# rikuu/Gap2Seq

Hardware: AMD Instinct MI355X
Metric: gaps filled/sec (whole node), k=31 synthetic 3 Mbp DBG (higher is better)
Workload: dtype u32

## Files before the change

gap2seq_amd/csrc/d3_device.h:

```cpp
#pragma once
#include <hip/hip_runtime_api.h>
#include <stdint.h>

#include "d2_device.h"
#include "fill_device.h"

#define G2S_D3_BLOCK_VARS 16u
#define G2S_RAND_BLOCK 4096u
#define G2S_RAND_WINDOW 160u
#define G2S_D3_TABLE_BUDGET (8u << 20)

#define G2S_D3_UNHANDLED 0x1u
#define G2S_D3_BUDGET 0x2u
#define G2S_D3_ANOMALY 0x4u

namespace g2s {

struct D3Gap {
  uint64_t arena_off;
  int32_t skip_thr;
  uint16_t lmf;
  uint8_t kind;
  uint8_t pad;
};
// ... 32 lines not shown
static_assert(sizeof(D3Var) == 64 && sizeof(D3Trace) == 32, "record layouts");

struct D3Summary {
  uint32_t status, unhandled, n_var, anomalies;
  unsigned long long host_items, host_segs, host_rnd;
  uint32_t handoff_waves, tiles;
  uint64_t table_entries, block_entries;
  uint64_t draws_min, draws_spread, draws_total;
  uint64_t xA, sA, xB, sB, xD, sD, segs, fill_bytes;
  uint32_t seg_gaps, filled;
  uint32_t rand_state[31];
  uint32_t trace_waves;
  uint32_t big_gaps;
  uint32_t traced_gaps;
  uint32_t spec_gaps;
};
static_assert(sizeof(D3Summary) <= 512, "the lap stamps live at byte 512 of the summary's slot");

struct RandTables {
  const uint32_t* hi = nullptr;
  const uint32_t* mid = nullptr;
  const uint32_t* lane = nullptr;
};
void rand_tables_host(uint32_t* hi , uint32_t* mid , uint32_t* lane );

struct D3Work {
  uint32_t* ginfo = nullptr;
  uint32_t* dmin = nullptr;
  uint32_t* dspread = nullptr;
  uint32_t* base = nullptr;
// ... 62 lines not shown
                     const D3Gap* dgaps, const SubRec* sub, const char* lastch_up, const char* lastch_dn,
                     const RandTables& rt, uint32_t* rnd_all ,
                     uint64_t rnd_capacity, void* results ,
                     char* arena , const D3Side& side ,
                     void* summary_host ,
                     bool summary_is_clean ,
                     uint32_t* clean_words ,
                     hipEvent_t ev_chain = nullptr ,
                     hipEvent_t ev_d2 = nullptr ,
                     hipEvent_t ev_stop = nullptr );

hipError_t test_d3_tables(const uint32_t* segs, uint32_t nsegs, int32_t n_len, int32_t len0, int32_t len1, uint32_t start_seg,
                          const uint32_t* rnd, uint64_t rnd_cap, uint32_t base, uint32_t R, uint32_t dmin, uint32_t dspread,
                          uint16_t* entries, uint8_t* bad, uint32_t* anomalies);

}
```

gap2seq_amd/csrc/d3_device.hip:

```cpp
#include "sync_debug.h"
#include <hip/hip_runtime.h>
#include <hip/hip_ext.h>

#include <algorithm>
#include <cstddef>
#include <cstdlib>
#include <cstring>
#include <mutex>
#include <set>
#include <vector>

#include "../../include/g2s.h"
#include "d3_device.h"
#include "envcache.hpp"

namespace {

using g2s::D3Gap;
using g2s::D3Params;
using g2s::D3Summary;
using g2s::D3Work;

__device__ __forceinline__ uint32_t uni(uint32_t x) { return (uint32_t)__builtin_amdgcn_readfirstlane((int)x); }

// ... 38 lines not shown
  x = sat_add(x, (uint32_t)__builtin_amdgcn_update_dpp(0, (int)x, 0x143, 0xC, 0xF, false));
  return x;
}
__device__ __forceinline__ uint32_t dpp_sum(uint32_t x) { return (uint32_t)__builtin_amdgcn_readlane((int)dpp_scan_add(x), 63); }
__device__ __forceinline__ unsigned long long wave_add64(unsigned long long v) {
  const unsigned long long lo = dpp_sum((uint32_t)v & 0xFFFFFFu), mid = dpp_sum((uint32_t)(v >> 24) & 0xFFFFFFu), hi = dpp_sum((uint32_t)(v >> 48));
  return lo + (mid << 24) + (hi << 48);
}

__device__ __forceinline__ uint32_t d3_classify_body(const D3Params& P, const D3Work& W, const GapOut* __restrict__ outs,
                                                     const D3Gap* __restrict__ dgaps, uint32_t first, uint32_t stride,
                                                     uint32_t* l_gi, uint32_t* l_dm, uint32_t* l_ds, int32_t* l_sk,
                                                     unsigned long long* red, bool one_wg) {
  const uint32_t n = P.n;
  unsigned long long xA = 0, sA = 0, xB = 0, sB = 0, xD = 0, sD = 0, segs = 0;
  uint32_t unhandled = 0, seg_gaps = 0, big = 0, traced = 0, spec = 0;
  for (uint32_t i = first; i < n; i += stride) {
    const D3Gap dg = dgaps[i];
    const GapOut& go = outs[i];
    const uint32_t flags = go.flags, n_states = go.n_states, n_right = go.n_right, x_right = go.x_right, x_left = go.x_left;
    const uint32_t x_sub = go.x_sub, n_sub = go.n_sub, nseg_b = go.stat[3], dflags = go.dflags, stop0 = go.stop[0], stop1 = go.stop[1];
    const int c_count = go.c_count, n_len = go.n_len, len0 = go.len[0], len1 = go.len[1], reached_j = go.reached_j, count_s = go.count_s;
    const uint32_t n_xl = go.n_xl;
    const uint64_t sub_off = go.sub_off;
    uint32_t gi = 0, dmin = 0, spread = 0;
    if (dg.kind != 0) gi = GI_BAD;
    else {
      if (flags & (G2S_DEV_OVERFLOW_A | G2S_DEV_OVERFLOW_B)) unhandled++;
      else if ((uint64_t)n_states > P.max_states || (uint64_t)n_right > P.max_states) gi = GI_MEM;
      else {
        xA += x_right; sA += n_right; xB += x_left; sB += n_states; xD += x_sub; sD += n_sub;
        segs += nseg_b;
        seg_gaps++;
        if (flags & G2S_DEV_BIG) big++;
        if (dflags & G2S_DEVA_TRACED) traced++;
        if (dflags & G2S_DEVA_SPEC) spec++;
        const bool phase_d = c_count > 0 && n_len > 0;
        const bool by_host = phase_d && !(dflags & (G2S_DEVA_ANALYSED | G2S_DEVA_D2_PENDING));
        const int cnt = (phase_d && !P.skip_confident && P.all_paths) ? count_s : c_count;
        if (cnt > 0 && (!P.unique_paths || cnt == 1)) gi |= GI_FILLED;
        if (n_len > 0) gi |= ((uint32_t)reached_j & 0xFFu) << 8;
        if (phase_d) {
          gi |= GI_PHASE_D;
          if (by_host) gi |= GI_HOST;
          int lo_d = 0x7FFFFFFF, hi_d = 0;
#pragma unroll
          for (int q = 0; q < 2; q++) {
            if (q >= n_len) continue;
            const uint32_t sw = q ? stop1 : stop0;
            const int lq = q ? len1 : len0;
            int lo = (int)(sw & 0xFFFFu), hi = (int)(sw >> 16);
            if (lo > hi || hi > (int)dg.lmf) { lo = 0; hi = (int)dg.lmf; }
            lo_d = min(lo_d, 1 + lq - hi);
            hi_d = max(hi_d, 1 + lq - lo);
          }
          lo_d = max(lo_d, 1);
          hi_d = max(hi_d, lo_d);
          dmin = (uint32_t)lo_d;
          spread = (uint32_t)(hi_d - lo_d);
// ... 10 lines not shown
    uint4 h0;
    const uint64_t ao = P.arena_base + dg.arena_off, sa = (uint64_t)(i / P.group_size) * P.sub_region + sub_off;
    h0.x = (uint32_t)ao; h0.y = (uint32_t)(ao >> 32); h0.z = (uint32_t)sa; h0.w = (uint32_t)(sa >> 32);
    ((uint4*)&W.tdesc[i])[0] = h0;
    (void)n_xl;
  }
  xA = wave_add64(xA); sA = wave_add64(sA); xB = wave_add64(xB); sB = wave_add64(sB); xD = wave_add64(xD); sD = wave_add64(sD);
  segs = wave_add64(segs);
  const unsigned long long cnts = wave_add64(((unsigned long long)unhandled << 32) | seg_gaps);
  big = dpp_sum(big);
  if ((threadIdx.x & 63u) == 0u && big) atomicAdd(&W.sum->big_gaps, big);
  traced = dpp_sum(traced);
  if ((threadIdx.x & 63u) == 0u && traced) atomicAdd(&W.sum->traced_gaps, traced);
  spec = dpp_sum(spec);
  if ((threadIdx.x & 63u) == 0u && spec) atomicAdd(&W.sum->spec_gaps, spec);
  const uint32_t wave = threadIdx.x >> 6, nwaves = blockDim.x >> 6;
  if ((threadIdx.x & 63u) == 0u) {
    unsigned long long* r = red + wave * 8u;
    r[0] = xA; r[1] = sA; r[2] = xB; r[3] = sB; r[4] = xD; r[5] = sD; r[6] = segs; r[7] = cnts;
  }
  __syncthreads();
  unsigned long long tot = 0;
  if (threadIdx.x < 8u) for (uint32_t w = 0; w < nwaves; w++) tot += red[w * 8u + threadIdx.x];
  unsigned long long all_cnts = 0;
  for (uint32_t w = 0; w < nwaves; w++) all_cnts += red[w * 8u + 7u];
  D3Summary* S = W.sum;
  if (threadIdx.x < 7u) {
    unsigned long long* dst = (unsigned long long*)&S->xA + threadIdx.x;
    if (one_wg) *dst = tot; else if (tot) atomicAdd(dst, tot);
  } else if (threadIdx.x == 7u) {
// ... 852 lines not shown
  (void)d3_classify_body(P, W, outs, dgaps, blockIdx.x * 256u + threadIdx.x, gridDim.x * 256u, nullptr, nullptr, nullptr, nullptr, red, false);
  (void)d3_handoff_body<true>(P, W, outs, sub, rnd, capacity, side, blockIdx.x * 256u + (threadIdx.x & ~63u), nullptr, nullptr, nullptr, nullptr);
  if ((threadIdx.x & 63u) == 0u) {
    asm volatile("s_waitcnt vmcnt(0)" ::: "memory");
    const unsigned int done = atomicAdd(&S->handoff_waves, 1u) + 1u;
    if (done == gridDim.x * 4u) {
      const unsigned long long items = atomicAdd(&S->host_items, 0ull);
      const uint32_t anomalies = atomicAdd(&S->anomalies, 0u), unhandled = atomicAdd(&S->unhandled, 0u);
      S->status = unhandled ? G2S_D3_UNHANDLED : 0u;
      __hip_atomic_store(side.count, (items & 0x7FFFFFFFFFFFFFFFull) | ((unsigned long long)((anomalies || unhandled) ? 1u : 0u) << 63),
                         __ATOMIC_RELEASE, __HIP_MEMORY_SCOPE_SYSTEM);
    }
  }
}
#define D3_BACK_TAB 24576u
__global__ __launch_bounds__(1024) void g2s_d3_back(const D3Params P, const D3Work W, const GapOut* __restrict__ outs,
                                                    const SubRec* __restrict__ sub, const uint32_t* __restrict__ Wd, uint64_t capacity,
                                                    const g2s::D3Side side) {
  __shared__ uint32_t total_dev;
  __shared__ unsigned long long lcur[3];
  if (threadIdx.x < 3u) lcur[threadIdx.x] = 0ull;
  __shared__ uint16_t ltab[D3_BACK_TAB];
  __shared__ uint32_t ltoff[1025], ldvar[1025];
  D3Summary* S = W.sum;
  if (threadIdx.x == 0) stamp(W, 8);
  const uint32_t status = S->status, V = S->n_var;
  const uint64_t T = S->table_entries;
  if (status) {
    if (threadIdx.x == 0) __hip_atomic_store(side.count, 1ull << 63, __ATOMIC_RELEASE, __HIP_MEMORY_SCOPE_SYSTEM);
    return;
// ... 31 lines not shown
  for (uint32_t i0 = (threadIdx.x >> 6) * 64u; i0 < P.n; i0 += 1024u)
    (void)d3_handoff_body<false>(P, W, outs, sub, Wd + 31, capacity, side, i0, in_lds ? ldvar : nullptr, in_lds ? ltab : nullptr,
                          in_lds ? ltoff : nullptr, lcur);
  __syncthreads();
  if (threadIdx.x == 0) {
    stamp(W, 11);
    const unsigned long long items = lcur[0];
    S->host_items = items; S->host_segs = lcur[1]; S->host_rnd = lcur[2];
    const uint32_t anomalies = atomicAdd(&S->anomalies, 0u);
    __hip_atomic_store(side.count, (items & 0x7FFFFFFFFFFFFFFFull) | ((unsigned long long)(anomalies ? 1u : 0u) << 63), __ATOMIC_RELEASE,
                       __HIP_MEMORY_SCOPE_SYSTEM);
    stamp(W, 12);
  }
}

template <int NW>
__global__ __launch_bounds__(64 * NW) void g2s_d3_trace(const D3Params P, const D3Work W, GapOut* __restrict__ outs,
                                                   const SubRec* __restrict__ sub, const char* __restrict__ chu,
                                                   const char* __restrict__ chd, const uint32_t* __restrict__ rnd,
                                                   uint64_t capacity, g2s_result* __restrict__ results,
                                                   char* __restrict__ arena, uint32_t* __restrict__ summary_host,
                                                   const g2s::D3Side side, uint32_t* __restrict__ clean_words ) {
  extern __shared__ __attribute__((aligned(16))) uint32_t lds[];
  D3Summary* S = W.sum;
  const uint32_t i = blockIdx.x;
  constexpr int NT = 64 * NW;
  const int tid = (int)threadIdx.x, lane = tid & 63;
  const bool w0 = tid < 64;
#ifdef G2S_SYNC_DEBUG
  auto wg_sync = [&]() { if constexpr (NW > 1) __syncthreads(); else { g2s_sync_jitter(0xD3u); g2s_wait_all(); asm volatile("s_waitcnt lgkmcnt(0)" ::: "memory"); __builtin_amdgcn_wave_barrier(); } };
#else
  auto wg_sync = [&]() { if constexpr (NW > 1) __syncthreads(); else { asm volatile("s_waitcnt lgkmcnt(0)" ::: "memory"); __builtin_amdgcn_wave_barrier(); } };
#endif
  SegW* segs = (SegW*)lds;
  static_assert(sizeof(g2s_result) == 112, "g2s_result layout");
  unsigned long long* laps = (unsigned long long*)((char*)W.sum + 512);
  const unsigned long long tk0 = P.laps ? wall_clock64() : 0ull;
  unsigned long long tk1 = 0, tk2 = 0, tk3 = 0, hops = 0, tkm = 0;
  if (P.laps && i == 0 && tid == 0) laps[13] = tk0;
  const uint32_t status = uni(S->status);
  g2s::D3Trace td;
  {
    const uint4 h0 = ((const uint4*)&W.tdesc[i])[0], h1 = ((const uint4*)&W.tdesc[i])[1];
    td.arena_off = (uint64_t)uni(h0.x) | ((uint64_t)uni(h0.y) << 32);
    td.sub_at = (uint64_t)uni(h0.z) | ((uint64_t)uni(h0.w) << 32);
    td.gi = uni(h1.x); td.off = uni(h1.y); td.want = uni(h1.z);
    td.lmf = (uint16_t)(uni(h1.w) & 0xFFFFu); td.nsegs = (uint16_t)(uni(h1.w) >> 16);
  }
  struct {
    uint32_t flags, dflags, start_seg, start_t, sub_vertices, sub_edges, top_level;
    int32_t c_count, n_len, len[2], reached_j, count_s;
  } go;
  {
    const GapOut& g = outs[i];
    go.top_level = uni(g.top_level);
    go.flags = uni(g.flags); go.dflags = uni(g.dflags); go.start_seg = uni(g.start_seg); go.start_t = uni(g.start_t);
    go.sub_vertices = uni(g.sub_vertices); go.sub_edges = uni(g.sub_edges);
    go.c_count = (int32_t)uni((uint32_t)g.c_count); go.n_len = (int32_t)uni((uint32_t)g.n_len);
    go.len[0] = (int32_t)uni((uint32_t)g.len[0]); go.len[1] = (int32_t)uni((uint32_t)g.len[1]);
    go.reached_j = (int32_t)uni((uint32_t)g.reached_j); go.count_s = (int32_t)uni((uint32_t)g.count_s);
  }
  bool d2_lost = false;
  if ((go.dflags & G2S_DEVA_D2_PENDING) && !(go.dflags & (G2S_DEVA_RUNS | G2S_DEVA_D2_FAILED)) && !P.skip_confident) {
    uint32_t v = go.dflags;
    for (uint32_t spin = 0; spin < (1u << 22) && !(v & (G2S_DEVA_RUNS | G2S_DEVA_D2_FAILED)); spin++) {
      __builtin_amdgcn_s_sleep(8);
      v = uni(__hip_atomic_load(&outs[i].dflags, __ATOMIC_ACQUIRE, __HIP_MEMORY_SCOPE_AGENT));
    }
    __builtin_amdgcn_fence(__ATOMIC_ACQUIRE, "agent");
    go.dflags = v;
    go.sub_vertices = uni(__hip_atomic_load(&outs[i].sub_vertices, __ATOMIC_RELAXED, __HIP_MEMORY_SCOPE_AGENT));
    go.sub_edges = uni(__hip_atomic_load(&outs[i].sub_edges, __ATOMIC_RELAXED, __HIP_MEMORY_SCOPE_AGENT));
    if (!(v & (G2S_DEVA_RUNS | G2S_DEVA_D2_FAILED))) d2_lost = true;
  }
  if ((go.dflags & G2S_DEVA_D2_PENDING) && (go.dflags & G2S_DEVA_D2_FAILED) && !(td.gi & GI_HOST) && (td.gi & GI_PHASE_D)) d2_lost = true;
  uint32_t gsp_all = 0, gsp_sent = 0;
  auto leave = [&](uint32_t fill_len) {
    if (!w0) return;
    uint32_t last = 0;
    if (lane == 0) {
      if (P.laps) {
        const unsigned long long tk4 = wall_clock64();
        atomicMax(&laps[14], tk1 ? tk1 - tk0 : 0ull); atomicMax(&laps[15], tk2 ? tk2 - tk1 : 0ull);
        atomicMax(&laps[16], tk3 ? tk3 - tk2 : 0ull); atomicMax(&laps[17], ((tk4 - tk0) << 24) | ((td.gi & GI_HOST) ? 1ull << 23 : 0ull) | (unsigned long long)(i & 0x7FFFFFu)); atomicMax(&laps[18], tk4);
        atomicMax(&laps[19], ((tk2 ? tk2 - tk1 : 0ull) << 32) | (hops << 16) | (tkm ? tkm - tk1 : 0ull));
        if ((P.laps >> 4) == i + 1u) { laps[26] = tk0; laps[27] = tk1; laps[28] = tkm; laps[29] = tk2; laps[30] = tk3; laps[31] = tk4; }
      }
      const uint32_t c = i & 63u, n = gridDim.x;
// ... 16 lines not shown
    const unsigned long long c1 = __hip_atomic_load(cl + 1, __ATOMIC_RELAXED, __HIP_MEMORY_SCOPE_AGENT);
    summary_host[lane] = s0;
    summary_host[64 + lane] = s1;
    ((unsigned long long*)(summary_host + 256 + 32 * lane))[0] = c0;
    ((unsigned long long*)(summary_host + 256 + 32 * lane))[1] = c1;
    if (P.self_clean) {
      src[lane] = 0u; src[64 + lane] = 0u;
      ((unsigned long long*)(src + 256 + 32 * lane))[0] = 0ull;
      ((unsigned long long*)(src + 256 + 32 * lane))[1] = 0ull;
    }
    if (P.self_clean && clean_words && lane < 32) clean_words[lane] = 0u;
    if (P.laps && lane == 0) { asm volatile("s_waitcnt vmcnt(0)" ::: "memory"); laps[25] = wall_clock64(); }
  };
  if (status) { leave(0u); return; }
  if (d2_lost) {
    if (tid == 0) { atomicAdd(&S->anomalies, 1u); arena[td.arena_off + td.lmf] = '\0'; }
    asm volatile("s_waitcnt vmcnt(0)" ::: "memory");
    leave(0u);
    return;
  }
  const uint32_t gi = td.gi;
  if ((go.dflags & G2S_DEVA_TRACED) && !(gi & (GI_BAD | GI_SKIPPED | GI_MEM | GI_HOST)) && (gi & GI_PHASE_D)) {
    asm volatile("s_waitcnt vmcnt(0)" ::: "memory");
    leave((go.top_level >> 16) - (go.top_level & 0xFFFFu));
    return;
  }
  const bool spec = (go.dflags & G2S_DEVA_SPEC) != 0u && W.spec_text != nullptr && !(gi & (GI_BAD | GI_SKIPPED | GI_MEM | GI_HOST)) && (gi & GI_PHASE_D);
  const int spec_stop = (int)(go.top_level & 0xFFFFu), spec_len = (int)(go.top_level >> 16);
  const unsigned long long spec_chain = spec ? ((unsigned long long)uni(outs[i].stat[6]) | ((unsigned long long)uni(outs[i].stat[7]) << 32)) : 0ull;
  struct { uint16_t lmf; } dg = {td.lmf};
  const uint64_t abs_off = td.arena_off;
// ... 43 lines not shown
    rw[16] = go.sub_vertices; rw[18] = go.sub_edges;
    if (by_runs) {
      const uint4 o0 = ((const uint4*)&W.d2out[i])[0], o1 = ((const uint4*)&W.d2out[i])[1];
      runs = W.d2runs + 2ull * uni(o0.x);
      n_runs = uni(o0.y);
      rw[8] = uni(o0.z); rw[10] = uni(o0.w); rw[12] = uni(o1.x); rw[14] = uni(o1.y); rw[16] = uni(o1.z); rw[18] = uni(o1.w);
    }
  }
  if (!phase_d) {
    if (tid == 0) buf[dg.lmf] = '\0';
    finish(0u);
    leave(0u);
    return;
  }
  if (gi & GI_HOST) {
    const uint32_t it = uni(W.host_slot[i]);
    if (it != 0xFFFFFFFFu) {
      const g2s::D3HostItem* hp = &W.hitems[it];
      const uint64_t so = (uint64_t)uni((uint32_t)hp->seg_off) | ((uint64_t)uni((uint32_t)(hp->seg_off >> 32)) << 32);
      const uint64_t ro = (uint64_t)uni((uint32_t)hp->rnd_off) | ((uint64_t)uni((uint32_t)(hp->rnd_off >> 32)) << 32);
      const uint32_t ns = uni(hp->n_segs), want = uni(hp->draws);
      const GapOut& g = outs[i];
      if ((uint32_t)tid < sizeof(GapOut) / 4u) ((uint32_t*)&side.outs[it])[tid] = ((const uint32_t*)&g)[tid];
      const uint4* src = (const uint4*)(sub + td.sub_at);
      uint4* dst = (uint4*)(side.segs + so);
      for (uint32_t w = (uint32_t)tid; w < 2u * ns; w += (uint32_t)NT) dst[w] = src[w];
      for (uint32_t w = (uint32_t)tid; w < (want + 8u) / 8u; w += (uint32_t)NT) {
        uint32_t pk8 = 0u;
#pragma unroll
        for (uint32_t x = 0; x < 8u; x++) {
          const uint32_t at = 8u * w + x;
          if (at <= want) pk8 |= ((rnd[td.off + at] >> 1) % 12u) << (4u * x);
        }
        side.rnd[ro + w] = pk8;
      }
      __threadfence_system();
// ... 489 lines not shown
  hipLaunchKernelGGL(g2s_d3_blocks, dim3(256), dim3(256), 0, st, W);
  hipLaunchKernelGGL(g2s_d3_groupfn, dim3(std::min(256u, (P.R0 + 256u) / 256u)), dim3(256), 0, st, W, P.R0, group_fn);
  return hipGetLastError();
}
hipError_t launch_d3_sharded_trace(hipStream_t st, const D3Params& P, const D3Work& W, const GapOut* outs, const SubRec* sub,
                                   const char* lastch_up, const char* lastch_dn, uint32_t* rnd_all, uint64_t rnd_capacity,
                                   void* results, char* arena, const D3Side& side, void* summary_host, hipEvent_t ev_d2) {
  if (P.n == 0) return hipSuccess;
  hipLaunchKernelGGL(g2s_d3_chain, dim3(1), dim3(1024), 0, st, W, rnd_all, P.base0, P.d_in);
  if (ev_d2) { const hipError_t e2 = hipStreamWaitEvent(st, ev_d2, 0); if (e2 != hipSuccess) return e2; }
  hipLaunchKernelGGL(g2s_d3_handoff, dim3((P.n + 63u) / 64u), dim3(64), 0, st, P, W, outs, sub, rnd_all + 31, rnd_capacity, side);
  const size_t lds = (size_t)P.seg_cap * (sizeof(SegRec) + 16) + (size_t)P.map_cap * 8 + 16;
  hipError_t e = hipFuncSetAttribute((const void*)g2s_d3_trace<1>, hipFuncAttributeMaxDynamicSharedMemorySize, (int)lds);
  if (e != hipSuccess) return e;
  hipLaunchKernelGGL(g2s_d3_trace<1>, dim3(P.n), dim3(64), lds, st, P, W, const_cast<GapOut*>(outs), sub, lastch_up, lastch_dn, rnd_all + 31, rnd_capacity,
                     (g2s_result*)results, arena, (uint32_t*)summary_host, side, (uint32_t*)nullptr);
  return hipGetLastError();
}

hipError_t launch_d3(hipStream_t st, const D3Params& P, const D3Work& W, const GapDev* gaps, const GapOut* outs,
                     const D3Gap* dgaps, const SubRec* sub, const char* lastch_up, const char* lastch_dn,
                     const RandTables& rt, uint32_t* rnd_all, uint64_t rnd_capacity, void* results, char* arena,
                     const D3Side& side, void* summary_host, bool summary_is_clean, uint32_t* clean_words, hipEvent_t ev_chain,
                     hipEvent_t ev_d2, hipEvent_t ev_stop) {
  if (P.n == 0) return hipSuccess;
  (void)gaps;
  (void)rt;
  static_assert(sizeof(D3Summary) <= 1024, "summary slot");
  hipError_t e = summary_is_clean ? hipSuccess : hipMemsetAsync(W.sum, 0, 1024 + 64 * 128, st);
  if (e != hipSuccess) return e;
  const bool short_list = P.n <= D3_FRONT_GAPS;
  if (P.restart) {
    if (ev_d2) { e = hipStreamWaitEvent(st, ev_d2, 0); if (e != hipSuccess) return e; }
    hipLaunchKernelGGL(g2s_d3_restart, dim3((P.n + 255u) / 256u), dim3(256), 0, st, P, W, outs, dgaps, sub, rnd_all + 31, rnd_capacity, side);
  } else if (short_list) hipLaunchKernelGGL(g2s_d3_front, dim3(1), dim3(1024), 0, st, P, W, outs, dgaps);
  else {
    hipLaunchKernelGGL(g2s_d3_classify, dim3((P.n + 255u) / 256u), dim3(256), 0, st, P, W, outs, dgaps);
    launch_scan(st, P, W, outs);
  }
  if (!P.restart) { e = launch_tables(st, P, W, sub, rnd_all, rnd_capacity); if (e != hipSuccess) return e; }
  if (ev_d2 && short_list && !P.restart) { e = hipStreamWaitEvent(st, ev_d2, 0); if (e != hipSuccess) return e; }
  if (P.restart) (void)ev_chain;
  else if (short_list) {
    hipLaunchKernelGGL(g2s_d3_back, dim3(1), dim3(1024), 0, st, P, W, outs, sub, rnd_all, rnd_capacity, side);
    if (ev_chain) { e = hipEventRecord(ev_chain, st); if (e != hipSuccess) return e; }
  } else {
    hipLaunchKernelGGL(g2s_d3_blocks, dim3(256), dim3(256), 0, st, W);
    hipLaunchKernelGGL(g2s_d3_chain, dim3(1), dim3(1024), 0, st, W, rnd_all, 0u, 0u);
    if (ev_chain) { e = hipEventRecord(ev_chain, st); if (e != hipSuccess) return e; }
    if (ev_d2) { e = hipStreamWaitEvent(st, ev_d2, 0); if (e != hipSuccess) return e; }
    hipLaunchKernelGGL(g2s_d3_handoff, dim3((P.n + 63u) / 64u), dim3(64), 0, st, P, W, outs, sub, rnd_all + 31, rnd_capacity, side);
  }
  const size_t lds = (size_t)P.seg_cap * (sizeof(SegRec) + 16) + (size_t)P.map_cap * 8 + 16;
  const char* waves_s = GENV("G2S_TRACE_WAVES");
  const int waves_env = waves_s ? atoi(waves_s) : 0;
  const bool four = waves_env ? waves_env == 4 : P.n <= 768u;
  e = hipFuncSetAttribute(four ? (const void*)g2s_d3_trace<4> : (const void*)g2s_d3_trace<1>, hipFuncAttributeMaxDynamicSharedMemorySize, (int)lds);
  if (e != hipSuccess) return e;
  if (ev_stop != nullptr) {
    if (four)
      hipExtLaunchKernelGGL(g2s_d3_trace<4>, dim3(P.n), dim3(256), (uint32_t)lds, st, nullptr, ev_stop, 0u, P, W, const_cast<GapOut*>(outs), sub, lastch_up, lastch_dn,
                            rnd_all + 31, rnd_capacity, (g2s_result*)results, arena, (uint32_t*)summary_host, side, clean_words);
    else
      hipExtLaunchKernelGGL(g2s_d3_trace<1>, dim3(P.n), dim3(64), (uint32_t)lds, st, nullptr, ev_stop, 0u, P, W, const_cast<GapOut*>(outs), sub, lastch_up, lastch_dn,
                            rnd_all + 31, rnd_capacity, (g2s_result*)results, arena, (uint32_t*)summary_host, side, clean_words);
    return hipGetLastError();
  }
  if (four)
    hipLaunchKernelGGL(g2s_d3_trace<4>, dim3(P.n), dim3(256), lds, st, P, W, const_cast<GapOut*>(outs), sub, lastch_up, lastch_dn, rnd_all + 31, rnd_capacity,
                       (g2s_result*)results, arena, (uint32_t*)summary_host, side, clean_words);
  else
    hipLaunchKernelGGL(g2s_d3_trace<1>, dim3(P.n), dim3(64), lds, st, P, W, const_cast<GapOut*>(outs), sub, lastch_up, lastch_dn, rnd_all + 31, rnd_capacity,
                       (g2s_result*)results, arena, (uint32_t*)summary_host, side, clean_words);
  return hipGetLastError();
}

}
```

gap2seq_amd/csrc/g2s_api.hip:

```cpp
#include <hip/hip_runtime.h>
#include <cstdarg>
#include <sys/prctl.h>
#include <pthread.h>
#include <sched.h>
#include <time.h>

#include <algorithm>
#include <atomic>
#include <chrono>
#include <cstdio>
#include <cstdlib>
#include <condition_variable>
#include <cstring>
#include <functional>
#include <mutex>
#include <string>
#include <thread>
#include <vector>

#include "../../include/g2s.h"
#include "../../include/g2s_test.h"
#include "envcache.hpp"
#include "d2_device.h"
#include "d3_device.h"
// ... 4761 lines not shown
}

extern "C" int g2s_test_d3_tables(int device, const uint32_t* segs, uint32_t n_segs, int32_t n_len, int32_t len0, int32_t len1,
                                  uint32_t start_seg, const uint32_t* rnd, uint64_t rnd_cap, uint32_t base, uint32_t R, uint32_t dmin,
                                  uint32_t dspread, uint16_t* entries, uint8_t* bad, uint32_t* anomalies) {
  if ((!segs && n_segs) || (!rnd && rnd_cap) || !entries || !bad || !anomalies || n_segs > 0xFFFFu || n_len < 1 || n_len > 2 ||
      (uint64_t)R + 1u > (uint64_t)G2S_D3_TABLE_BUDGET)
    return fail(G2S_ERR_ARG, "g2s_test_d3_tables: bad argument");
  int ndev = 0;
  if (hipGetDeviceCount(&ndev) != hipSuccess || device < 0 || device >= ndev) return fail(G2S_ERR_NO_DEVICE, "no such device");
  HIP_TRY(hipSetDevice(device));
  HIP_TRY(test_d3_tables(segs, n_segs, n_len, len0, len1, start_seg, rnd, rnd_cap, base, R, dmin, dspread, entries, bad, anomalies));
  return G2S_OK;
}

extern "C" int g2s_test_rand_skip(uint32_t seed, uint64_t skip, uint32_t n, int32_t* out) {
  if (!out) return fail(G2S_ERR_ARG, "g2s_test_rand_skip: bad argument");
  GlibcRandStream st;
  st.seed(seed);
  st.skip(skip);
  st.ensure(n);
  for (uint32_t i = 0; i < n; i++) out[i] = st.value(i);
  return G2S_OK;
}
extern "C" int g2s_test_rand_stream(uint32_t seed, uint32_t skip, uint32_t n, int32_t* out) {
  if (!out) return fail(G2S_ERR_ARG, "g2s_test_rand_stream: bad argument");
  GlibcRandStream st;
  st.seed(seed);
  st.ensure(skip / 2 + 1);
  st.consume(skip / 2);
// ... 6 lines not shown
```

gap2seq_amd/lib.py:

```python
import ctypes as C
import os

G2S_OK = 0
G2S_ERR_IO = -2
G2S_ERR_NO_DEVICE = -3
G2S_ERR_STATE = -6
G2S_INVALID_NODE = 0xFFFFFFFF
G2S_MAX_PATHS = 2147483647 // 2 - 1
G2S_MAX_IN_FLIGHT = 3
G2S_GROUP_PER_SESSION = (1 << 64) - 1
G2S_GAP_SKIPPED = 0x1
G2S_GAP_Q7 = 0x2
G2S_GAP_MEM_EXCEEDED = 0x4
G2S_GAP_BACKTRACE_FAIL = 0x8
G2S_GAP_BAD_FLANK = 0x10
G2S_GAP_PHASE_D = 0x20


class G2SError(RuntimeError):
    def __init__(self, code, msg):
        super().__init__("g2s error %d: %s" % (code, msg))
        self.code = code


# ... 170 lines not shown
    "g2s_filter_reads_gaps_pool_mem": (C.c_int, [C.c_char_p, C.c_size_t, C.POINTER(g2s_filter_opts), C.POINTER(g2s_filter_gap),
                                                 C.c_size_t, C.c_int, C.c_int, C.c_int, C.POINTER(C.POINTER(g2s_read_pool)),
                                                 C.POINTER(C.c_int64), C.POINTER(g2s_filter_stats)]),
    "g2s_read_pool_free": (None, [C.POINTER(g2s_read_pool)]),
    "g2s_filter_last_error": (C.c_char_p, []),
    "g2s_device_count": (C.c_int, []),
    "g2s_synth_genome": (C.c_int, [C.c_uint64, C.c_uint32, C.c_uint64, C.POINTER(_VP)]),
    "g2s_synth_gaps": (C.c_int, [C.c_char_p, C.c_int, C.c_int, C.c_int, C.c_int, C.c_int, C.c_uint64,
                                 C.POINTER(_VP)]),
    "g2s_test_rand_skip": (C.c_int, [C.c_uint32, C.c_uint64, C.c_uint32, C.POINTER(C.c_int32)]),
    "g2s_test_rand_stream": (C.c_int, [C.c_uint32, C.c_uint32, C.c_uint32, C.POINTER(C.c_int32)]),
    "g2s_test_device_rand": (C.c_int, [C.c_int, C.c_uint32, C.c_uint64, C.c_uint32, C.POINTER(C.c_int32)]),
    "g2s_test_d3_tables": (C.c_int, [C.c_int, C.POINTER(C.c_uint32), C.c_uint32, C.c_int32, C.c_int32, C.c_int32, C.c_uint32,
                                     C.POINTER(C.c_uint32), C.c_uint64, C.c_uint32, C.c_uint32, C.c_uint32, C.c_uint32,
                                     C.POINTER(C.c_uint16), C.POINTER(C.c_uint8), C.POINTER(C.c_uint32)]),
    "g2s_test_post_closure": (C.c_int, [_VP, C.POINTER(g2s_params), C.POINTER(g2s_gap), C.c_uint32,
                                        C.POINTER(C.c_uint32), C.c_uint32, C.POINTER(C.c_uint64), C.c_int32, C.c_int32,
                                        C.POINTER(C.c_int32), C.c_int32, C.c_int32, C.c_uint32, C.c_uint64,
                                        C.POINTER(g2s_result), C.c_char_p]),
    "g2s_test_graph_tables": (C.c_int, [_VP, C.POINTER(C.c_uint32), C.POINTER(C.c_uint64)]),
    "g2s_test_post_segments": (C.c_int, [_VP, C.POINTER(g2s_params), C.POINTER(g2s_gap), C.c_uint32,
                                         C.POINTER(C.c_uint32), C.c_int32, C.c_int32, C.POINTER(C.c_int32), C.c_int32,
                                         C.c_int32, C.c_uint32, C.c_uint64, C.POINTER(g2s_result), C.c_char_p,
                                         C.POINTER(C.c_int32)]),
    "g2s_test_seg_expand": (C.c_int, [_VP, C.POINTER(g2s_params), C.POINTER(g2s_gap), C.c_uint32, C.POINTER(C.c_uint32),
                                      C.c_int32, C.POINTER(C.c_int32), C.c_int32, C.c_uint32, C.POINTER(C.c_uint32),
                                      C.c_uint32, C.POINTER(C.c_uint64)]),
    "g2s_test_worker_pool": (C.c_int, [C.c_int32, C.c_int32, C.c_int32]),
    "g2s_test_group_queue": (C.c_int, [C.c_int32, C.c_uint64, C.c_uint64, C.POINTER(C.c_int32)]),
    "g2s_test_group_queue_slow": (C.c_int, [C.c_int32, C.c_uint64, C.c_uint64, C.c_int32, C.c_uint32, C.POINTER(C.c_int32)]),
# ... 775 lines not shown
    out = (C.c_int32 * max(1, n))()
    _check(load_library().g2s_test_device_rand(device, seed, skip, n, out))
    return [out[i] for i in range(n)]


def test_d3_tables(device, segs, n_len, len0, len1, start_seg, rnd, base, R, dmin, dspread):
    flat = [w for s in segs for w in s]
    sa = (C.c_uint32 * max(1, len(flat)))(*flat)
    ra = (C.c_uint32 * max(1, len(rnd)))(*rnd)
    ent, bad, anom = (C.c_uint16 * (R + 1))(), (C.c_uint8 * (R + 1))(), C.c_uint32()
    _check(load_library().g2s_test_d3_tables(device, sa, len(segs), n_len, len0, len1, start_seg, ra, len(rnd), base, R, dmin,
                                             dspread, ent, bad, C.byref(anom)))
    return list(ent), list(bad), anom.value


def test_group_queue_slow(nworkers, n, group_size, slow_worker, slow_us):
    owner = (C.c_int32 * max(1, n))()
    _check(load_library().g2s_test_group_queue_slow(nworkers, n, group_size, slow_worker, slow_us, owner))
    return [owner[i] for i in range(n)]


def test_rand_skip(seed, skip, n):
    out = (C.c_int32 * max(1, n))()
    _check(load_library().g2s_test_rand_skip(seed, skip, n, out))
    return [out[i] for i in range(n)]


def test_rand_stream(seed, skip, n):
    out = (C.c_int32 * max(1, n))()
    _check(load_library().g2s_test_rand_stream(seed, skip, n, out))
# ... 196 lines not shown
```

Before: 3.154 million.

## Fold D3 back/chain stage and host handoff into the four-wave trace kernel

For small batches (up to 768 gaps, single group, no restart), the separate g2s_d3_back chain kernel is skipped. Each trace workgroup instead loads the per-variable table offsets and table into LDS, recomputes its own draw offset with a prefix walk, and allocates host handoff slots itself. The last gap writes the final draw total and RNG state, and a new handoff_gaps counter lets the last handoff block publish the host item count. This removes one kernel launch and a serial single-block pass, at the cost of every block redundantly scanning the prefix over all variables.

```diff
diff --git a/gap2seq_amd/csrc/d3_device.h b/gap2seq_amd/csrc/d3_device.h
--- a/gap2seq_amd/csrc/d3_device.h
+++ b/gap2seq_amd/csrc/d3_device.h
@@ -70,6 +70,7 @@
   uint32_t big_gaps;
   uint32_t traced_gaps;
   uint32_t spec_gaps;
+  uint32_t handoff_gaps;
 };
 static_assert(sizeof(D3Summary) <= 512, "the lap stamps live at byte 512 of the summary's slot");
 
@@ -162,4 +163,6 @@
                           const uint32_t* rnd, uint64_t rnd_cap, uint32_t base, uint32_t R, uint32_t dmin, uint32_t dspread,
                           uint16_t* entries, uint8_t* bad, uint32_t* anomalies);
 
+uint64_t d3_chain_launches();
+
 }
diff --git a/gap2seq_amd/csrc/d3_device.hip b/gap2seq_amd/csrc/d3_device.hip
--- a/gap2seq_amd/csrc/d3_device.hip
+++ b/gap2seq_amd/csrc/d3_device.hip
@@ -3,6 +3,7 @@
 #include <hip/hip_ext.h>
 
 #include <algorithm>
+#include <atomic>
 #include <cstddef>
 #include <cstdlib>
 #include <cstring>
@@ -76,7 +77,7 @@
                                                      unsigned long long* red, bool one_wg) {
   const uint32_t n = P.n;
   unsigned long long xA = 0, sA = 0, xB = 0, sB = 0, xD = 0, sD = 0, segs = 0;
-  uint32_t unhandled = 0, seg_gaps = 0, big = 0, traced = 0, spec = 0;
+  uint32_t unhandled = 0, seg_gaps = 0, big = 0, traced = 0, spec = 0, handoff = 0;
   for (uint32_t i = first; i < n; i += stride) {
     const D3Gap dg = dgaps[i];
     const GapOut& go = outs[i];
@@ -105,6 +106,7 @@
         if (phase_d) {
           gi |= GI_PHASE_D;
           if (by_host) gi |= GI_HOST;
+          if (by_host || (!P.skip_confident && (dflags & G2S_DEVA_D2_PENDING))) handoff++;
           int lo_d = 0x7FFFFFFF, hi_d = 0;
 #pragma unroll
           for (int q = 0; q < 2; q++) {
@@ -145,6 +147,8 @@
   if ((threadIdx.x & 63u) == 0u && traced) atomicAdd(&W.sum->traced_gaps, traced);
   spec = dpp_sum(spec);
   if ((threadIdx.x & 63u) == 0u && spec) atomicAdd(&W.sum->spec_gaps, spec);
+  handoff = dpp_sum(handoff);
+  if ((threadIdx.x & 63u) == 0u && handoff) atomicAdd(&W.sum->handoff_gaps, handoff);
   const uint32_t wave = threadIdx.x >> 6, nwaves = blockDim.x >> 6;
   if ((threadIdx.x & 63u) == 0u) {
     unsigned long long* r = red + wave * 8u;
@@ -1027,6 +1031,8 @@
   }
 }
 #define D3_BACK_TAB 24576u
+#define D3_CHAIN_GAPS 768u
+#define D3_CHAIN_ROOM 4096u
 __global__ __launch_bounds__(1024) void g2s_d3_back(const D3Params P, const D3Work W, const GapOut* __restrict__ outs,
                                                     const SubRec* __restrict__ sub, const uint32_t* __restrict__ Wd, uint64_t capacity,
                                                     const g2s::D3Side side) {
@@ -1088,13 +1094,15 @@
   }
 }
 
-template <int NW>
+template <int NW, bool CHAIN = false>
 __global__ __launch_bounds__(64 * NW) void g2s_d3_trace(const D3Params P, const D3Work W, GapOut* __restrict__ outs,
                                                    const SubRec* __restrict__ sub, const char* __restrict__ chu,
                                                    const char* __restrict__ chd, const uint32_t* __restrict__ rnd,
                                                    uint64_t capacity, g2s_result* __restrict__ results,
                                                    char* __restrict__ arena, uint32_t* __restrict__ summary_host,
-                                                   const g2s::D3Side side, uint32_t* __restrict__ clean_words ) {
+                                                   const g2s::D3Side side, uint32_t* __restrict__ clean_words ,
+                                                   uint32_t chain_room ) {
+  static_assert(!CHAIN || NW == 4, "the chain's loads are laid out for 256 threads");
   extern __shared__ __attribute__((aligned(16))) uint32_t lds[];
   D3Summary* S = W.sum;
   const uint32_t i = blockIdx.x;
@@ -1113,14 +1121,6 @@
   unsigned long long tk1 = 0, tk2 = 0, tk3 = 0, hops = 0, tkm = 0;
   if (P.laps && i == 0 && tid == 0) laps[13] = tk0;
   const uint32_t status = uni(S->status);
-  g2s::D3Trace td;
-  {
-    const uint4 h0 = ((const uint4*)&W.tdesc[i])[0], h1 = ((const uint4*)&W.tdesc[i])[1];
-    td.arena_off = (uint64_t)uni(h0.x) | ((uint64_t)uni(h0.y) << 32);
-    td.sub_at = (uint64_t)uni(h0.z) | ((uint64_t)uni(h0.w) << 32);
-    td.gi = uni(h1.x); td.off = uni(h1.y); td.want = uni(h1.z);
-    td.lmf = (uint16_t)(uni(h1.w) & 0xFFFFu); td.nsegs = (uint16_t)(uni(h1.w) >> 16);
-  }
   struct {
     uint32_t flags, dflags, start_seg, start_t, sub_vertices, sub_edges, top_level;
     int32_t c_count, n_len, len[2], reached_j, count_s;
@@ -1134,6 +1134,91 @@
     go.len[0] = (int32_t)uni((uint32_t)g.len[0]); go.len[1] = (int32_t)uni((uint32_t)g.len[1]);
     go.reached_j = (int32_t)uni((uint32_t)g.reached_j); go.count_s = (int32_t)uni((uint32_t)g.count_s);
   }
+  g2s::D3Trace td;
+  uint32_t c_dmin = 0, c_vr = 0, c_base = 0, c_V = 0, c_dev = 0, c_step = 0, c_ns = 0, c_handoff = 0;
+  uint64_t c_T = 0, c_draws_min = 0;
+  if constexpr (!CHAIN) {
+    const uint4 h0 = ((const uint4*)&W.tdesc[i])[0], h1 = ((const uint4*)&W.tdesc[i])[1];
+    td.arena_off = (uint64_t)uni(h0.x) | ((uint64_t)uni(h0.y) << 32);
+    td.sub_at = (uint64_t)uni(h0.z) | ((uint64_t)uni(h0.w) << 32);
+    td.gi = uni(h1.x); td.off = uni(h1.y); td.want = uni(h1.z);
+    td.lmf = (uint16_t)(uni(h1.w) & 0xFFFFu); td.nsegs = (uint16_t)(uni(h1.w) >> 16);
+  } else {
+    const uint32_t n = P.n;
+    const uint32_t toff_len = (n + 2u) & ~1u;
+    const uint32_t tab_room = chain_room > toff_len ? min(chain_room - toff_len, D3_CHAIN_ROOM) & ~1u : 0u;
+    uint16_t* ltoff = (uint16_t*)lds;
+    uint16_t* ltab = ltoff + toff_len;
+    const uint4 h0 = ((const uint4*)&W.tdesc[i])[0];
+    uint32_t gi_w = W.ginfo[i], dm_w = W.dmin[i], vr_w = W.vrank[i], bs_w = W.base[i], ns_w = outs[i].n_xl, V_w = S->n_var;
+    c_T = S->table_entries;
+    c_draws_min = S->draws_min;
+    uint32_t hg_w = S->handoff_gaps;
+    static_assert(D3_CHAIN_ROOM <= 8u * 2u * 256u && D3_CHAIN_GAPS <= 4u * 256u, "the unrolled loads below cover the room");
+    uint32_t tw[8], ow[4];
+    const uint32_t* tab32 = (const uint32_t*)W.tab;
+    const uint32_t tab_last = max(tab_room / 2u, 1u) - 1u;
+#pragma unroll
+    for (uint32_t q = 0; q < 8u; q++) tw[q] = tab32[min((uint32_t)tid + 256u * q, tab_last)];
+#pragma unroll
+    for (uint32_t q = 0; q < 4u; q++) ow[q] = W.var_toff[min((uint32_t)tid + 256u * q, n)];
+#pragma unroll
+    for (uint32_t q = 0; q < 8u; q++) { const uint32_t x = (uint32_t)tid + 256u * q; if (x < tab_room / 2u) ((uint32_t*)ltab)[x] = tw[q]; }
+#pragma unroll
+    for (uint32_t q = 0; q < 4u; q++) { const uint32_t x = (uint32_t)tid + 256u * q; if (x <= n) ltoff[x] = (uint16_t)ow[q]; }
+    td.arena_off = (uint64_t)uni(h0.x) | ((uint64_t)uni(h0.y) << 32);
+    td.sub_at = (uint64_t)uni(h0.z) | ((uint64_t)uni(h0.w) << 32);
+    td.gi = uni(gi_w); td.off = 0u; td.want = 0u;
+    td.lmf = (uint16_t)(td.gi >> 16);
+    c_ns = uni(ns_w);
+    td.nsegs = (uint16_t)min(c_ns, 0xFFFFu);
+    c_dmin = uni(dm_w); c_vr = uni(vr_w); c_base = uni(bs_w); c_V = uni(V_w); c_handoff = uni(hg_w);
+    c_T = (uint64_t)uni((uint32_t)c_T) | ((uint64_t)uni((uint32_t)(c_T >> 32)) << 32);
+    c_draws_min = (uint64_t)uni((uint32_t)c_draws_min) | ((uint64_t)uni((uint32_t)(c_draws_min >> 32)) << 32);
+    __syncthreads();
+    if (!status) {
+      const bool in_lds = c_T <= (uint64_t)tab_room && c_T <= 0xFFFFull && c_V <= n;
+      const uint32_t v0 = min(c_vr, c_V), var = GI_CLASS(td.gi) == 2u && v0 < c_V ? 1u : 0u;
+      const uint32_t v_end = i + 1u == n ? c_V : v0 + var;
+      uint32_t d = 0, dv = 0, d1 = 0;
+      if (in_lds) {
+        uint32_t t = ltoff[0];
+        for (uint32_t v = 0; v < v_end; v++) {
+          const uint32_t tn = ltoff[v + 1u];
+          if (v == v0) dv = d;
+          d += ltab[min(t + d, tab_room - 1u)];
+          if (v == v0) d1 = d;
+          t = tn;
+        }
+      } else {
+        for (uint32_t v = 0; v < v_end; v++) {
+          if (v == v0) dv = d;
+          d += W.tab[min((uint64_t)W.var_toff[v] + d, (uint64_t)G2S_D3_TABLE_BUDGET - 1u)];
+          if (v == v0) d1 = d;
+        }
+      }
+      if (v_end <= v0) dv = d;
+      c_dev = uni(dv);
+      c_step = var ? uni(d1) - c_dev : 0u;
+      td.off = c_base + c_dev;
+      td.want = c_dmin + c_step;
+      if (i + 1u == n && w0) {
+        const uint32_t d_all = uni(d);
+        const uint64_t total = c_draws_min + d_all;
+        if (lane == 0) {
+          W.dvar[c_V] = d_all;
+          __hip_atomic_store((unsigned long long*)&S->draws_total, (unsigned long long)total, __ATOMIC_RELAXED, __HIP_MEMORY_SCOPE_AGENT);
+        }
+        if (lane < 31) {
+          const uint32_t w = (rnd - 31)[total + (uint32_t)lane];
+          __hip_atomic_store(&S->rand_state[lane], w, __ATOMIC_RELAXED, __HIP_MEMORY_SCOPE_AGENT);
+          if (W.link) W.link[lane] = w;
+        }
+        __threadfence();
+      }
+    }
+    __syncthreads();
+  }
   bool d2_lost = false;
   if ((go.dflags & G2S_DEVA_D2_PENDING) && !(go.dflags & (G2S_DEVA_RUNS | G2S_DEVA_D2_FAILED)) && !P.skip_confident) {
     uint32_t v = go.dflags;
@@ -1146,6 +1231,49 @@
     go.sub_vertices = uni(__hip_atomic_load(&outs[i].sub_vertices, __ATOMIC_RELAXED, __HIP_MEMORY_SCOPE_AGENT));
     go.sub_edges = uni(__hip_atomic_load(&outs[i].sub_edges, __ATOMIC_RELAXED, __HIP_MEMORY_SCOPE_AGENT));
     if (!(v & (G2S_DEVA_RUNS | G2S_DEVA_D2_FAILED))) d2_lost = true;
+  }
+  uint32_t h_it = 0xFFFFFFFFu, h_ns = 0, h_want = 0;
+  uint64_t h_so = 0, h_ro = 0;
+  bool lost_counted = false;
+  if constexpr (CHAIN) {
+    const bool counts = (td.gi & GI_HOST) || ((td.gi & GI_PHASE_D) && !P.skip_confident && (go.dflags & G2S_DEVA_D2_PENDING));
+    if (!status && !d2_lost) {
+      if ((td.gi & GI_PHASE_D) && !P.skip_confident && (go.dflags & G2S_DEVA_D2_PENDING) && (go.dflags & G2S_DEVA_D2_FAILED)) td.gi |= GI_HOST;
+      if (td.gi & GI_HOST) {
+        __shared__ unsigned long long l_hand[3];
+        if (tid == 0) {
+          const uint32_t ns = c_ns, want = td.want;
+          unsigned long long it = atomicAdd(&S->host_items, 1ull);
+          const unsigned long long so = atomicAdd(&S->host_segs, (unsigned long long)ns);
+          const unsigned long long ro = atomicAdd(&S->host_rnd, ((unsigned long long)want + 8ull) / 8ull);
+          if (it >= side.cap_items || so + ns > side.cap_segs || ro + (want + 8ull) / 8ull > side.cap_rnd || (uint64_t)td.off + want + 1ull > capacity) {
+            atomicAdd(&S->anomalies, 1u);
+            it = 0xFFFFFFFFull;
+          } else {
+            uint32_t* hi = (uint32_t*)&side.items[it];
+            hi[0] = i; hi[1] = ns; hi[2] = (uint32_t)so; hi[3] = (uint32_t)(so >> 32); hi[4] = (uint32_t)ro; hi[5] = (uint32_t)(ro >> 32); hi[6] = want;
+            __threadfence_system();
+          }
+          l_hand[0] = it; l_hand[1] = so; l_hand[2] = ro;
+        }
+        __syncthreads();
+        h_it = uni((uint32_t)l_hand[0]);
+        h_so = (uint64_t)uni((uint32_t)l_hand[1]) | ((uint64_t)uni((uint32_t)(l_hand[1] >> 32)) << 32);
+        h_ro = (uint64_t)uni((uint32_t)l_hand[2]) | ((uint64_t)uni((uint32_t)(l_hand[2] >> 32)) << 32);
+        h_ns = c_ns; h_want = td.want;
+      }
+    }
+    if (tid == 0 && (counts || (c_handoff == 0u && i == 0u))) {
+      if (d2_lost && !status) { atomicAdd(&S->anomalies, 1u); lost_counted = true; }
+      asm volatile("s_waitcnt vmcnt(0)" ::: "memory");
+      const unsigned int done = counts ? atomicAdd(&S->handoff_waves, 1u) + 1u : 0u;
+      if (done == c_handoff) {
+        const unsigned long long items = atomicAdd(&S->host_items, 0ull);
+        const uint32_t anomalies = atomicAdd(&S->anomalies, 0u);
+        __hip_atomic_store(side.count, (items & 0x7FFFFFFFFFFFFFFFull) | ((unsigned long long)((anomalies || status) ? 1u : 0u) << 63),
+                           __ATOMIC_RELEASE, __HIP_MEMORY_SCOPE_SYSTEM);
+      }
+    }
   }
   if ((go.dflags & G2S_DEVA_D2_PENDING) && (go.dflags & G2S_DEVA_D2_FAILED) && !(td.gi & GI_HOST) && (td.gi & GI_PHASE_D)) d2_lost = true;
   uint32_t gsp_all = 0, gsp_sent = 0;
@@ -1192,7 +1320,7 @@
   };
   if (status) { leave(0u); return; }
   if (d2_lost) {
-    if (tid == 0) { atomicAdd(&S->anomalies, 1u); arena[td.arena_off + td.lmf] = '\0'; }
+    if (tid == 0) { if (!lost_counted) atomicAdd(&S->anomalies, 1u); arena[td.arena_off + td.lmf] = '\0'; }
     asm volatile("s_waitcnt vmcnt(0)" ::: "memory");
     leave(0u);
     return;
@@ -1266,12 +1394,12 @@
     return;
   }
   if (gi & GI_HOST) {
-    const uint32_t it = uni(W.host_slot[i]);
+    const uint32_t it = CHAIN ? h_it : uni(W.host_slot[i]);
     if (it != 0xFFFFFFFFu) {
-      const g2s::D3HostItem* hp = &W.hitems[it];
-      const uint64_t so = (uint64_t)uni((uint32_t)hp->seg_off) | ((uint64_t)uni((uint32_t)(hp->seg_off >> 32)) << 32);
-      const uint64_t ro = (uint64_t)uni((uint32_t)hp->rnd_off) | ((uint64_t)uni((uint32_t)(hp->rnd_off >> 32)) << 32);
-      const uint32_t ns = uni(hp->n_segs), want = uni(hp->draws);
+      const g2s::D3HostItem* hp = &W.hitems[CHAIN ? 0u : it];
+      const uint64_t so = CHAIN ? h_so : (uint64_t)uni((uint32_t)hp->seg_off) | ((uint64_t)uni((uint32_t)(hp->seg_off >> 32)) << 32);
+      const uint64_t ro = CHAIN ? h_ro : (uint64_t)uni((uint32_t)hp->rnd_off) | ((uint64_t)uni((uint32_t)(hp->rnd_off >> 32)) << 32);
+      const uint32_t ns = CHAIN ? h_ns : uni(hp->n_segs), want = CHAIN ? h_want : uni(hp->draws);
       const GapOut& g = outs[i];
       if ((uint32_t)tid < sizeof(GapOut) / 4u) ((uint32_t*)&side.outs[it])[tid] = ((const uint32_t*)&g)[tid];
       const uint4* src = (const uint4*)(sub + td.sub_at);
@@ -1791,9 +1919,12 @@
   hipError_t e = hipFuncSetAttribute((const void*)g2s_d3_trace<1>, hipFuncAttributeMaxDynamicSharedMemorySize, (int)lds);
   if (e != hipSuccess) return e;
   hipLaunchKernelGGL(g2s_d3_trace<1>, dim3(P.n), dim3(64), lds, st, P, W, const_cast<GapOut*>(outs), sub, lastch_up, lastch_dn, rnd_all + 31, rnd_capacity,
-                     (g2s_result*)results, arena, (uint32_t*)summary_host, side, (uint32_t*)nullptr);
+                     (g2s_result*)results, arena, (uint32_t*)summary_host, side, (uint32_t*)nullptr, 0u);
   return hipGetLastError();
 }
+
+static std::atomic<uint64_t> chain_launches{0};
+uint64_t d3_chain_launches() { return chain_launches.load(std::memory_order_relaxed); }
 
 hipError_t launch_d3(hipStream_t st, const D3Params& P, const D3Work& W, const GapDev* gaps, const GapOut* outs,
                      const D3Gap* dgaps, const SubRec* sub, const char* lastch_up, const char* lastch_dn,
@@ -1817,7 +1948,22 @@
   }
   if (!P.restart) { e = launch_tables(st, P, W, sub, rnd_all, rnd_capacity); if (e != hipSuccess) return e; }
   if (ev_d2 && short_list && !P.restart) { e = hipStreamWaitEvent(st, ev_d2, 0); if (e != hipSuccess) return e; }
+  const char* waves_s = GENV("G2S_TRACE_WAVES");
+  const int waves_env = waves_s ? atoi(waves_s) : 0;
+  const bool four = waves_env ? waves_env == 4 : P.n <= 768u;
+  const size_t lds = (size_t)P.seg_cap * (sizeof(SegRec) + 16) + (size_t)P.map_cap * 8 + 16;
+  bool chain_in_trace = false;
+  uint32_t chain_room = 0;
+  static_assert(D3_CHAIN_GAPS <= 768u, "g2s_d3_trace<4, true> is the four-wave kernel");
+  if (!P.restart && four && P.n <= D3_CHAIN_GAPS && ev_chain == nullptr && P.group_size >= P.n && !P.base0 && !P.R0 && !P.d_in) {
+    const char* back_s = GENV("G2S_D3_BACK");
+    chain_in_trace = !(back_s && atoi(back_s) != 0);
+    const char* room_s = GENV("G2S_TEST_CHAIN_ROOM");
+    chain_room = (uint32_t)std::min<size_t>(lds / 2u, 0x7FFFFFFFu);
+    if (room_s) chain_room = std::min(chain_room, (uint32_t)std::max(atoi(room_s), 0));
+  }
   if (P.restart) (void)ev_chain;
+  else if (chain_in_trace) (void)ev_chain;
   else if (short_list) {
     hipLaunchKernelGGL(g2s_d3_back, dim3(1), dim3(1024), 0, st, P, W, outs, sub, rnd_all, rnd_capacity, side);
     if (ev_chain) { e = hipEventRecord(ev_chain, st); if (e != hipSuccess) return e; }
@@ -1828,27 +1974,34 @@
     if (ev_d2) { e = hipStreamWaitEvent(st, ev_d2, 0); if (e != hipSuccess) return e; }
     hipLaunchKernelGGL(g2s_d3_handoff, dim3((P.n + 63u) / 64u), dim3(64), 0, st, P, W, outs, sub, rnd_all + 31, rnd_capacity, side);
   }
-  const size_t lds = (size_t)P.seg_cap * (sizeof(SegRec) + 16) + (size_t)P.map_cap * 8 + 16;
-  const char* waves_s = GENV("G2S_TRACE_WAVES");
-  const int waves_env = waves_s ? atoi(waves_s) : 0;
-  const bool four = waves_env ? waves_env == 4 : P.n <= 768u;
-  e = hipFuncSetAttribute(four ? (const void*)g2s_d3_trace<4> : (const void*)g2s_d3_trace<1>, hipFuncAttributeMaxDynamicSharedMemorySize, (int)lds);
+  e = hipFuncSetAttribute(chain_in_trace ? (const void*)g2s_d3_trace<4, true> : four ? (const void*)g2s_d3_trace<4> : (const void*)g2s_d3_trace<1>,
+                          hipFuncAttributeMaxDynamicSharedMemorySize, (int)lds);
   if (e != hipSuccess) return e;
+  if (chain_in_trace) {
+    chain_launches.fetch_add(1, std::memory_order_relaxed);
+    if (ev_stop != nullptr)
+      hipExtLaunchKernelGGL((g2s_d3_trace<4, true>), dim3(P.n), dim3(256), (uint32_t)lds, st, nullptr, ev_stop, 0u, P, W, const_cast<GapOut*>(outs), sub, lastch_up, lastch_dn,
+                            rnd_all + 31, rnd_capacity, (g2s_result*)results, arena, (uint32_t*)summary_host, side, clean_words, chain_room);
+    else
+      hipLaunchKernelGGL((g2s_d3_trace<4, true>), dim3(P.n), dim3(256), lds, st, P, W, const_cast<GapOut*>(outs), sub, lastch_up, lastch_dn, rnd_all + 31, rnd_capacity,
+                         (g2s_result*)results, arena, (uint32_t*)summary_host, side, clean_words, chain_room);
+    return hipGetLastError();
+  }
   if (ev_stop != nullptr) {
     if (four)
       hipExtLaunchKernelGGL(g2s_d3_trace<4>, dim3(P.n), dim3(256), (uint32_t)lds, st, nullptr, ev_stop, 0u, P, W, const_cast<GapOut*>(outs), sub, lastch_up, lastch_dn,
-                            rnd_all + 31, rnd_capacity, (g2s_result*)results, arena, (uint32_t*)summary_host, side, clean_words);
+                            rnd_all + 31, rnd_capacity, (g2s_result*)results, arena, (uint32_t*)summary_host, side, clean_words, 0u);
     else
       hipExtLaunchKernelGGL(g2s_d3_trace<1>, dim3(P.n), dim3(64), (uint32_t)lds, st, nullptr, ev_stop, 0u, P, W, const_cast<GapOut*>(outs), sub, lastch_up, lastch_dn,
-                            rnd_all + 31, rnd_capacity, (g2s_result*)results, arena, (uint32_t*)summary_host, side, clean_words);
+                            rnd_all + 31, rnd_capacity, (g2s_result*)results, arena, (uint32_t*)summary_host, side, clean_words, 0u);
     return hipGetLastError();
   }
   if (four)
     hipLaunchKernelGGL(g2s_d3_trace<4>, dim3(P.n), dim3(256), lds, st, P, W, const_cast<GapOut*>(outs), sub, lastch_up, lastch_dn, rnd_all + 31, rnd_capacity,
-                       (g2s_result*)results, arena, (uint32_t*)summary_host, side, clean_words);
+                       (g2s_result*)results, arena, (uint32_t*)summary_host, side, clean_words, 0u);
   else
     hipLaunchKernelGGL(g2s_d3_trace<1>, dim3(P.n), dim3(64), lds, st, P, W, const_cast<GapOut*>(outs), sub, lastch_up, lastch_dn, rnd_all + 31, rnd_capacity,
-                       (g2s_result*)results, arena, (uint32_t*)summary_host, side, clean_words);
+                       (g2s_result*)results, arena, (uint32_t*)summary_host, side, clean_words, 0u);
   return hipGetLastError();
 }
 
diff --git a/gap2seq_amd/csrc/g2s_api.hip b/gap2seq_amd/csrc/g2s_api.hip
--- a/gap2seq_amd/csrc/g2s_api.hip
+++ b/gap2seq_amd/csrc/g2s_api.hip
@@ -4799,6 +4799,8 @@
   return G2S_OK;
 }
 
+extern "C" uint64_t g2s_test_d3_chain_launches(void) { return d3_chain_launches(); }
+
 extern "C" int g2s_test_rand_skip(uint32_t seed, uint64_t skip, uint32_t n, int32_t* out) {
   if (!out) return fail(G2S_ERR_ARG, "g2s_test_rand_skip: bad argument");
   GlibcRandStream st;
diff --git a/gap2seq_amd/lib.py b/gap2seq_amd/lib.py
--- a/gap2seq_amd/lib.py
+++ b/gap2seq_amd/lib.py
@@ -208,6 +208,7 @@
     "g2s_test_d3_tables": (C.c_int, [C.c_int, C.POINTER(C.c_uint32), C.c_uint32, C.c_int32, C.c_int32, C.c_int32, C.c_uint32,
                                      C.POINTER(C.c_uint32), C.c_uint64, C.c_uint32, C.c_uint32, C.c_uint32, C.c_uint32,
                                      C.POINTER(C.c_uint16), C.POINTER(C.c_uint8), C.POINTER(C.c_uint32)]),
+    "g2s_test_d3_chain_launches": (C.c_uint64, []),
     "g2s_test_post_closure": (C.c_int, [_VP, C.POINTER(g2s_params), C.POINTER(g2s_gap), C.c_uint32,
                                         C.POINTER(C.c_uint32), C.c_uint32, C.POINTER(C.c_uint64), C.c_int32, C.c_int32,
                                         C.POINTER(C.c_int32), C.c_int32, C.c_int32, C.c_uint32, C.c_uint64,
@@ -1013,6 +1014,10 @@
     return list(ent), list(bad), anom.value
 
 
+def test_d3_chain_launches():
+    return int(load_library().g2s_test_d3_chain_launches())
+
+
 def test_group_queue_slow(nworkers, n, group_size, slow_worker, slow_us):
     owner = (C.c_int32 * max(1, n))()
     _check(load_library().g2s_test_group_queue_slow(nworkers, n, group_size, slow_worker, slow_us, owner))
```

New measurement: 3.255 million (median of 6 runs). +3.2%, better.
